# BornToDeath/h264-h265-to-jpeg

Hardware: AMD Instinct MI355X
Metric: 1080p H.265 I-frames/sec → JPEG at 1/2/4/8 MI355X; achieved HBM GB/s vs peak (higher is better)
Workload: dtype u8

## Files before the change

### h264-h265-to-jpeg_amd/csrc/host/cabac.h

```cpp
#pragma once
#include <cstdint>

namespace h2j {

#ifdef H2J_CABAC_COUNT
extern thread_local unsigned long long g_bins_ctx, g_bins_byp;
#define H2J_COUNT(v, n) (v += (n))
#else
#define H2J_COUNT(v, n) ((void)0)
#endif

#pragma GCC visibility push(hidden)
extern const uint8_t kCabacLps[64][4];
extern const uint8_t kCabacTransLps[64];
extern const uint8_t kCabacRenorm[32];
extern const uint16_t kCabacNextMps[128];
extern const uint16_t kCabacNextLps[128];
extern const uint8_t kCabacLpsByState[128][8];
typedef uint64_t CabacState;
extern const uint64_t kCabacWord[128];

extern const uint64_t kCabacNextMpsW[128];
extern const uint64_t kCabacNextLpsW[128];
#pragma GCC visibility pop


inline uint8_t cabac_init_state(int m, int n, int qp) {
    if (qp < 0) qp = 0;
    if (qp > 51) qp = 51;
    int pre = ((m * qp) >> 4) + n;
    if (pre < 1) pre = 1;
    if (pre > 126) pre = 126;
    int mps = pre <= 63 ? 0 : 1;
    int st = mps ? pre - 64 : 63 - pre;
    return static_cast<uint8_t>((st << 1) | mps);
}
inline CabacState cabac_init_word(int m, int n, int qp) { return kCabacWord[cabac_init_state(m, n, qp)]; }

template <bool kInlineRefill>
class CabacT {
public:
    void init(const uint8_t* p, const uint8_t* end) {
        cur_ = p;
        end_ = end;
        range_ = 510;
        value_ = 0;
        for (int i = 0; i < 4; i++) value_ = (value_ << 8) | (cur_ < end_ ? *cur_++ : 0u);
        bits_ = 32 - 9;
    }
    __attribute__((always_inline)) inline int decision(CabacState& ctx) {
        H2J_COUNT(g_bins_ctx, 1);
        const uint64_t w = ctx;
        const unsigned st = static_cast<unsigned>(w >> 32);
        const uint32_t lps = static_cast<uint32_t>(w >> ((range_ >> 3) & 24)) & 0xffu;
        const uint32_t rmps = range_ - lps;
        const uint64_t scaled = static_cast<uint64_t>(rmps) << bits_;
        const uint32_t msh = (rmps >> 8) ^ 1u;
        uint32_t r = rmps << msh, sh = msh;
        const uint32_t lsh = static_cast<uint32_t>(__builtin_clz(lps)) - 23u;
        const uint32_t lr = lps << lsh;
        uint64_t nx = kCabacNextMpsW[st];
        const uint64_t nl = kCabacNextLpsW[st];
        uint64_t v = value_;
        const uint64_t vl = value_ - scaled;
        uint32_t is_lps = 0;
#if defined(__x86_64__)
        __asm__("cmpq %[sc], %[v]\n\t"
                "cmovaeq %[vl], %[v]\n\t"
                "cmovael %[lr], %[r]\n\t"
                "cmovael %[ls], %[sh]\n\t"
                "cmovaeq %[nl], %[nx]\n\t"
                "setae %b[il]"
                : [v] "+r"(v), [r] "+r"(r), [sh] "+r"(sh), [nx] "+r"(nx), [il] "+q"(is_lps)
                : [sc] "r"(scaled), [vl] "r"(vl), [lr] "r"(lr), [ls] "r"(lsh), [nl] "r"(nl)
                : "cc");
#else
        is_lps = v >= scaled ? 1u : 0u;
        v = is_lps ? vl : v;
        r = is_lps ? lr : r;
        sh = is_lps ? lsh : sh;
        nx = is_lps ? nl : nx;
#endif
        value_ = v;
        range_ = r;
        bits_ -= static_cast<int>(sh);
        ctx = nx;
        if (bits_ < 0) refill();
        return static_cast<int>((st & 1) ^ is_lps);
    }
    __attribute__((always_inline)) int bypass_b() {
        H2J_COUNT(g_bins_byp, 1);
        if (--bits_ < 0) refill();
        const uint64_t scaled = static_cast<uint64_t>(range_) << bits_;
        const bool one = value_ >= scaled;
        value_ -= one ? scaled : 0;
        return one;
    }
    __attribute__((always_inline)) uint32_t bypass_batch_b(int k) {
        H2J_COUNT(g_bins_byp, k);
        if (bits_ < k) refill();
        const int sh = bits_ - k;
        const uint64_t v = value_ >> sh;
        const uint32_t q = static_cast<uint32_t>(v / range_);
        value_ -= (static_cast<uint64_t>(q) * range_) << sh;
        bits_ = sh;
        return q;
    }
    __attribute__((always_inline)) uint32_t bypass_peek_b(int k) {
        if (bits_ < k) refill();
        return static_cast<uint32_t>((value_ >> (bits_ - k)) / range_);
    }
    __attribute__((always_inline)) void bypass_skip_b(int n, uint32_t top) {
        H2J_COUNT(g_bins_byp, n);
        const int sh = bits_ - n;
        value_ -= (static_cast<uint64_t>(top) * range_) << sh;
        bits_ = sh;
    }
    __attribute__((always_inline)) uint32_t bypass_bits_b(int n) {
        if (n <= 2) {
            uint32_t v = 0;
            for (int i = 0; i < n; i++) v = (v << 1) | static_cast<uint32_t>(bypass());
            return v;
        }
        if (n <= 24) return bypass_batch(n);
        const uint32_t hi = bypass_batch(n - 16);
        return (hi << 16) | bypass_batch(16);
    }
    __attribute__((always_inline)) int terminate_b() {
        range_ -= 2;
        const uint64_t scaled = static_cast<uint64_t>(range_) << bits_;
        if (value_ >= scaled) return 1;
        if (range_ < 256) {
            range_ <<= 1;
            if (--bits_ < 0) refill();
// ... 64 lines not shown
```

### h264-h265-to-jpeg_amd/csrc/host/hevc_parser.cpp

```cpp
#include <algorithm>
#include <array>
#include <atomic>
#include <cstdlib>
#include <cstring>
#include <memory>
#include <thread>
#include <vector>

#include "bitstream.h"
#include "cabac.h"
#include "job.h"

namespace h2j {
#ifdef H2J_CORO
extern thread_local void (*g_h2j_yield)();
#endif
namespace {

enum {
    C_SAO_MERGE = 0, C_SAO_TYPE = 1, C_SPLIT_CU = 2, C_TQ_BYPASS = 5, C_PART_MODE = 6,
    C_PREV_INTRA = 7, C_CHROMA_MODE = 8, C_SPLIT_TF = 9, C_CBF_LUMA = 12, C_CBF_CHROMA = 14,
    C_TSKIP = 18, C_LAST_X = 20, C_LAST_Y = 38, C_CSBF = 56, C_SIG = 60, C_GT1 = 104,
    C_GT2 = 128, C_QP_DELTA = 134, C_CQO_FLAG = 136, C_CQO_IDX = 137, NUM_CTX = 138
};

const uint8_t kInitI[NUM_CTX] = {
    153, 200, 139, 141, 157, 154, 184, 184, 63, 153, 138, 138, 111, 141, 94, 138, 182, 154,
    139, 139,
    110, 110, 124, 125, 140, 153, 125, 127, 140, 109, 111, 143, 127, 111, 79, 108, 123, 63,
    110, 110, 124, 125, 140, 153, 125, 127, 140, 109, 111, 143, 127, 111, 79, 108, 123, 63,
    91, 171, 134, 141,
    111, 111, 125, 110, 110, 94, 124, 108, 124, 107, 125, 141, 179, 153, 125, 107, 125, 141,
    179, 153, 125, 107, 125, 141, 179, 153, 125, 140, 139, 182, 182, 152, 136, 152, 136, 153,
    136, 139, 111, 136, 139, 111, 141, 111,
    140, 92, 137, 138, 140, 152, 138, 139, 153, 74, 149, 92, 139, 107, 122, 152, 140, 179, 166,
    182, 140, 227, 122, 197,
    138, 153, 136, 167, 152, 152,
    154, 154,
    154, 154};

struct Sps {
    bool valid = false;
    int chroma_format_idc = 0, width = 0, height = 0;
    int conf_l = 0, conf_r = 0, conf_t = 0, conf_b = 0;
    int bit_depth = 8, bit_depth_c = 8, log2_max_poc_lsb = 4;
    int num_reorder_pics = 0;
    int log2_min_cb = 3, log2_ctb = 4, log2_min_tb = 2, log2_max_tb = 5, max_th_depth_intra = 0;
    int scaling_list_enabled = 0;
    uint8_t sl[4][6][64];
    uint8_t sl_dc[4][6];
    int sao = 0, pcm = 0, pcm_bd = 8, pcm_bd_c = 8, log2_min_pcm = 0, log2_max_pcm = 0, pcm_lf_disabled = 0;
    int num_st_rps = 0;
    int st_num_delta[65];
    int long_term_present = 0, num_lt_sps = 0, temporal_mvp = 0, strong_intra_smoothing = 0;
    int profile_idc = 0;
    int ts_rotation = 0, ts_context = 0, implicit_rdpcm = 0, explicit_rdpcm = 0, ext_precision = 0;
    int smoothing_disabled = 0, high_prec_offsets = 0, persistent_rice = 0, bypass_alignment = 0;
};

struct Pps {
    bool valid = false;
    int sps_id = 0, dependent_slices = 0, output_flag_present = 0, num_extra_bits = 0, sign_hiding = 0;
    int init_qp = 26, transform_skip = 0, cu_qp_delta = 0, diff_cu_qp_delta_depth = 0;
    int cb_qp_offset = 0, cr_qp_offset = 0, slice_chroma_qp_present = 0, transquant_bypass = 0;
    int tiles = 0, wpp = 0, ntc = 1, ntr = 1, uniform = 1, lf_across_tiles = 1;
    int col_w[64], row_h[64];
    int lf_across_slices = 0, deblock_override = 0, deblock_disabled = 0, beta_offset = 0, tc_offset = 0;
    int sl_present = 0;
    uint8_t sl[4][6][64];
    uint8_t sl_dc[4][6];
    int slice_header_ext = 0;
    int log2_max_ts = 2, cross_component = 0, cqo_list_enabled = 0, sao_scale_luma = 0, sao_scale_chroma = 0;
    int cqo_depth = 0, cqo_len_minus1 = 0, cb_qo[6] = {0, 0, 0, 0, 0, 0}, cr_qo[6] = {0, 0, 0, 0, 0, 0};
};

struct SliceHdr {
    int first_in_pic = 0, dependent = 0, address = 0, slice_addr_rs = 0, pps_id = 0, type = 0;
    int sao_luma = 0, sao_chroma = 0, qp_delta = 0, cb_qp_offset = 0, cr_qp_offset = 0;
    int deblock_disabled = 0, beta_offset = 0, tc_offset = 0, lf_across_slices = 0, slice_qp = 26;
    int cu_chroma_qp_offset_enabled = 0;
    std::vector<uint32_t> entry;
};

const uint8_t kSlIntra[64] = {
    16, 16, 16, 16, 16, 16, 16, 16, 16, 16, 17, 16, 17, 16, 17, 18, 17, 18, 18, 17, 18, 21,
    19, 20, 21, 20, 19, 21, 24, 22, 22, 24, 24, 22, 22, 24, 25, 25, 27, 30, 27, 25, 25, 29,
    31, 35, 35, 31, 29, 36, 41, 44, 41, 36, 47, 54, 54, 47, 65, 70, 65, 88, 88, 115};
const uint8_t kSlInter[64] = {
    16, 16, 16, 16, 16, 16, 16, 16, 16, 16, 17, 17, 17, 17, 17, 18, 18, 18, 18, 18, 18, 20,
    20, 20, 20, 20, 20, 20, 24, 24, 24, 24, 24, 24, 24, 24, 25, 25, 25, 25, 25, 25, 25, 28,
    28, 28, 28, 28, 28, 33, 33, 33, 33, 33, 41, 41, 41, 41, 54, 54, 54, 71, 71, 91};

void sl_default(uint8_t sl[4][6][64], uint8_t dc[4][6]) {
    for (int m = 0; m < 6; m++) {
        std::memset(sl[0][m], 16, 16);
        for (int s = 1; s < 4; s++) {
            std::memcpy(sl[s][m], m < 3 ? kSlIntra : kSlInter, 64);
            dc[s][m] = 16;
        }
// ... 266 lines not shown
    p.cr_qp_offset = b.se();
    if (p.cb_qp_offset < -12 || p.cb_qp_offset > 12 || p.cr_qp_offset < -12 || p.cr_qp_offset > 12) return -1;
    p.slice_chroma_qp_present = static_cast<int>(b.u(1));
    b.u(1);
    b.u(1);
    p.transquant_bypass = static_cast<int>(b.u(1));
    p.tiles = static_cast<int>(b.u(1));
    p.wpp = static_cast<int>(b.u(1));
    if (p.tiles) {
        const uint32_t ntc = b.ue(), ntr = b.ue();
        if (ntc > 63 || ntr > 63) return -1;
        p.ntc = static_cast<int>(ntc) + 1;
        p.ntr = static_cast<int>(ntr) + 1;
        p.uniform = static_cast<int>(b.u(1));
        if (!p.uniform) {
            for (int i = 0; i < p.ntc - 1; i++) {
                const uint32_t v = b.ue();
                if (v >= 512) return -1;
                p.col_w[i] = static_cast<int>(v) + 1;
            }
            for (int i = 0; i < p.ntr - 1; i++) {
                const uint32_t v = b.ue();
                if (v >= 512) return -1;
                p.row_h[i] = static_cast<int>(v) + 1;
            }
        }
        p.lf_across_tiles = static_cast<int>(b.u(1));
    }
    p.lf_across_slices = static_cast<int>(b.u(1));
    if (b.u(1)) {
        p.deblock_override = static_cast<int>(b.u(1));
        p.deblock_disabled = static_cast<int>(b.u(1));
        if (!p.deblock_disabled) {
            const int bo = b.se(), to = b.se();
            if (bo < -6 || bo > 6 || to < -6 || to > 6) return -1;
            p.beta_offset = bo * 2;
            p.tc_offset = to * 2;
        }
    }
    p.sl_present = static_cast<int>(b.u(1));
    if (p.sl_present) {
        sl_default(p.sl, p.sl_dc);
        parse_scaling_list(b, p.sl, p.sl_dc);
    }
    b.u(1);
    b.ue();
    p.slice_header_ext = static_cast<int>(b.u(1));
    if (b.u(1)) {
        const int range = static_cast<int>(b.u(1));
        b.u(7);
        if (range && sps.profile_idc == 4) {
            if (p.transform_skip) {
                const uint32_t v = b.ue();
                if (v > 3) return -1;
                p.log2_max_ts = static_cast<int>(v) + 2;
            }
            p.cross_component = static_cast<int>(b.u(1));
            p.cqo_list_enabled = static_cast<int>(b.u(1));
            if (p.cqo_list_enabled) {
                p.cqo_depth = static_cast<int>(std::min<uint32_t>(b.ue(), 64u));
                const uint32_t len = b.ue();
                if (len > 5) return -1;
                p.cqo_len_minus1 = static_cast<int>(len);
                for (uint32_t i = 0; i <= len; i++) {
                    p.cb_qo[i] = std::max(-128, std::min(128, b.se()));
                    p.cr_qo[i] = std::max(-128, std::min(128, b.se()));
                }
            }
            const uint32_t sl = b.ue(), sc = b.ue();
            const uint32_t lim = sps.bit_depth > 10 ? static_cast<uint32_t>(sps.bit_depth - 10) : 0u;
            if (sl > lim || sc > lim) return -1;
            p.sao_scale_luma = static_cast<int>(sl);
            p.sao_scale_chroma = static_cast<int>(sc);
        }
    }
    if (b.overrun()) return -1;
    p.valid = true;
    return 0;
}

uint8_t g_scan_diag[4][64][2], g_scan_hor[4][64][2], g_scan_ver[4][64][2];
uint8_t g_scan_inv[3][4][64];
uint16_t g_scan_off[3][4][16];
uint8_t g_diag_pos4[16];
uint8_t g_diag_pos8[64];
uint8_t g_sigctx[2][4][3][4][2][16];
bool g_scans_ready = false;

void init_scans() {
    if (g_scans_ready) return;
    for (int l = 0; l < 4; l++) {
        int bs = 1 << l, i = 0, x = 0, y = 0;
        while (i < bs * bs) {
            while (y >= 0) {
                if (x < bs && y < bs) {
                    g_scan_diag[l][i][0] = static_cast<uint8_t>(x);
                    g_scan_diag[l][i][1] = static_cast<uint8_t>(y);
                    i++;
                }
                y--;
                x++;
            }
            y = x;
            x = 0;
        }
        i = 0;
        for (y = 0; y < bs; y++)
            for (x = 0; x < bs; x++, i++) {
                g_scan_hor[l][i][0] = static_cast<uint8_t>(x);
                g_scan_hor[l][i][1] = static_cast<uint8_t>(y);
            }
        i = 0;
        for (x = 0; x < bs; x++)
            for (y = 0; y < bs; y++, i++) {
                g_scan_ver[l][i][0] = static_cast<uint8_t>(x);
                g_scan_ver[l][i][1] = static_cast<uint8_t>(y);
            }
    }
    for (int si = 0; si < 3; si++)
        for (int l = 0; l < 4; l++) {
            const uint8_t(*sc)[64][2] = si == 0 ? g_scan_diag : (si == 1 ? g_scan_hor : g_scan_ver);
            for (int i = 0; i < (1 << (2 * l)); i++)
                g_scan_inv[si][l][sc[l][i][1] * (1 << l) + sc[l][i][0]] = static_cast<uint8_t>(i);
        }
    for (int c = 0; c < 2; c++)
        for (int lsb = 0; lsb < 4; lsb++)
            for (int si = 0; si < 3; si++)
                for (int pc = 0; pc < 4; pc++)
                    for (int sb = 0; sb < 2; sb++)
                        for (int nn = 0; nn < 16; nn++) {
                            const uint8_t(*sc)[64][2] = si == 0 ? g_scan_diag : (si == 1 ? g_scan_hor : g_scan_ver);
                            const int log2n = lsb + 2, xp = sc[2][nn][0], yp = sc[2][nn][1];
                            int sigCtx;
                            if (log2n == 2) {
                                static const uint8_t m[16] = {0, 1, 4, 5, 2, 3, 4, 5, 6, 6, 8, 8, 7, 7, 8, 8};
                                sigCtx = m[(yp << 2) + xp];
                            } else if (!sb && xp + yp == 0) {
                                sigCtx = 0;
                            } else {
                                if (pc == 0) sigCtx = (xp + yp == 0) ? 2 : (xp + yp < 3) ? 1 : 0;
                                else if (pc == 1) sigCtx = (yp == 0) ? 2 : (yp == 1) ? 1 : 0;
                                else if (pc == 2) sigCtx = (xp == 0) ? 2 : (xp == 1) ? 1 : 0;
                                else sigCtx = 2;
                                if (c == 0) {
                                    if (sb) sigCtx += 3;
                                    sigCtx += (log2n == 3) ? ((si == 0) ? 9 : 15) : 21;
                                } else {
                                    sigCtx += (log2n == 3) ? 9 : 12;
                                }
                            }
                            g_sigctx[c][lsb][si][pc][sb][nn] = static_cast<uint8_t>(C_SIG + (c == 0 ? sigCtx : 27 + sigCtx));
                        }
    for (int si = 0; si < 3; si++) {
        const uint8_t(*sc)[64][2] = si == 0 ? g_scan_diag : (si == 1 ? g_scan_hor : g_scan_ver);
        for (int l = 0; l < 4; l++)
            for (int i = 0; i < 16; i++) g_scan_off[si][l][i] = static_cast<uint16_t>(sc[2][i][1] * (4 << l) + sc[2][i][0]);
    }
    for (int i = 0; i < 16; i++) g_diag_pos4[i] = static_cast<uint8_t>(g_scan_diag[2][i][1] * 4 + g_scan_diag[2][i][0]);
    for (int i = 0; i < 64; i++) g_diag_pos8[i] = static_cast<uint8_t>(g_scan_diag[3][i][1] * 8 + g_scan_diag[3][i][0]);
    g_scans_ready = true;
}

int chroma_qp_table(int qpi) {
    static const int t[14] = {29, 30, 31, 32, 33, 33, 34, 34, 35, 35, 36, 36, 37, 37};
    if (qpi < 30) return qpi;
    if (qpi > 43) return qpi - 6;
    return t[qpi - 30];
}

class HevcParser {
public:
    explicit HevcParser(FrameJob& job) : job_(&job), ctbs_(&job.ctbs) {}
    HevcParser(const HevcParser& proto, FrameJob& job) : HevcParser(proto) {
        job_ = &job;
        ctbs_ = &job.ctbs;
        bind_maps();
    }
    HevcParser(const HevcParser& proto, bool share_maps) : HevcParser(proto) {
        (void)share_maps;
        ctbs_ = proto.ctbs_;
    }
    int run(const uint8_t* data, size_t size, int threads);

private:
    HevcParser(const HevcParser&) = default;
    FrameJob* job_;
    std::vector<h2j_ctb>* ctbs_;
    Sps sps_[16];
    Pps pps_[64];
    const Sps* s_ = nullptr;
    const Pps* p_ = nullptr;
    std::vector<SliceHdr> sh_;
    std::vector<uint8_t> rbsp_;
    std::vector<uint8_t> slice_data_;
    int W = 0, H = 0, log2ctb = 0, ctbs = 0, ctbW = 0, ctbH = 0, nctb = 0, mw = 0, mh = 0;
    int qpbd = 0;
    std::vector<int8_t> qp_store_;
    std::vector<uint8_t> ipm_store_, ctd_store_;
    std::vector<int> addr_store_, slice_store_;
    int8_t* qp_ = nullptr;
    uint8_t *ipm_ = nullptr, *ctd_ = nullptr;
    int *ctb_addr_rs_ = nullptr, *ctb_slice_ = nullptr;
    void bind_maps() {
        qp_ = qp_store_.data();
        ipm_ = ipm_store_.data();
        ctd_ = ctd_store_.data();
        ctb_addr_rs_ = addr_store_.data();
        ctb_slice_ = slice_store_.data();
    }
    std::vector<int> rs2ts_, ts2rs_, tile_id_, col_bd_;
    const SliceHdr* cur_ = nullptr;
    int cur_idx_ = 0;
    Cabac cc_;
    const uint8_t* end_ = nullptr;
    CabacState ctx_[NUM_CTX], ctx_wpp_[NUM_CTX], ctx_ds_[NUM_CTX];
    int stat_[4] = {0, 0, 0, 0}, stat_wpp_[4] = {0, 0, 0, 0}, stat_ds_[4] = {0, 0, 0, 0};
    bool rext_ = false;
    bool have_ds_ = false;
    int qp_y_ = 0, qg_pred_ = 0, qpd_val_ = 0, last_cu_qp_ = 0;
    bool is_qpd_coded_ = false, first_qg_ = true;
    bool cqo_coded_ = false;
    int cu_qo_cb_ = 0, cu_qo_cr_ = 0;
    int cu_bypass_ = 0;
    int cu_tu_begin_ = 0;
    int err_ = 0;

    int parse_slice_header(BitReader& b, int nal_type, SliceHdr& sh, const SliceHdr* prev);
    bool setup_picture();
    bool setup_tiles();
    int decode_slice_data(int shi, const uint8_t* p, const uint8_t* end);
    struct WppRows;
    int decode_wpp_row(int shi, int row, const uint8_t* p, const uint8_t* end, WppRows& w);
    int run_wpp(const std::vector<uint8_t>& seg, const std::vector<uint32_t>& sub, int threads);
    int decode_tile(int shi, int ts0, int ts1, bool last, const uint8_t* p, const uint8_t* end);
    int run_tiles(const std::vector<uint8_t>& seg, const std::vector<uint32_t>& sub, int threads);
    void merge_parts(const std::vector<FrameJob>& part);
    void ctb_start_contexts(int rs, int ts, bool first);
    void init_contexts(int qp) {
        for (int i = 0; i < NUM_CTX; i++) {
            int iv = kInitI[i];
            ctx_[i] = cabac_init_word((iv >> 4) * 5 - 45, ((iv & 15) << 3) - 16, qp);
        }
        std::memset(stat_, 0, sizeof(stat_));
    }
    bool same_region(int xc, int yc, int xn, int yn) const {
        if (xn < 0 || yn < 0 || xn >= W || yn >= H) return false;
        if (((xn ^ xc) | (yn ^ yc)) >> log2ctb == 0) return true;
        int cn = (yn >> log2ctb) * ctbW + (xn >> log2ctb);
        int cc = (yc >> log2ctb) * ctbW + (xc >> log2ctb);
        if (tile_id_[rs2ts_[cn]] != tile_id_[rs2ts_[cc]] || ctb_slice_[cn] < 0) return false;
        return ctb_addr_rs_[cn] == ctb_addr_rs_[cc];
    }
    void qg_start(int xq, int yq);
    void parse_sao(int rx, int ry);
    void coding_quadtree(int x0, int y0, int log2cb, int depth);
    void coding_unit(int x0, int y0, int log2cb);
    void transform_tree(int x0, int y0, int xb, int yb, int log2n, int depth, int blk, int max_depth,
                        int intra_split, int pcb, int pcr, int cm, int cux, int cuy, int log2cb);
    void transform_unit(int x0, int y0, int xb, int yb, int log2n, int blk, int cbf_l, int cbf_cb,
                        int cbf_cr, int cm, int cux, int cuy, int log2cb);
    template <bool RExt>
    void residual(int log2n, int c, int mode, h2j_tu& tu);
    void emit_tu(int x, int y, int log2n, int c, int mode, uint8_t flags, bool cbf, int pred_mode_for_scan);
    void split_ctb_records(size_t first);
    std::vector<h2j_tu> chroma_tmp_;
    uint8_t edge_flags(int x0, int y0) const;
    void pcm_sample(int x0, int y0, int log2cb);
    int qp_wrap(int x) const {
        const int m = 52 + qpbd;
        if (static_cast<unsigned>(x) < static_cast<unsigned>(2 * m)) return x >= m ? x - m : x;
        return x % m;
    }
    static void fill_rows(uint8_t* p, int stride, int rows, int w, uint8_t v) {
        const uint64_t v8 = 0x0101010101010101ull * v;
        for (int y = 0; y < rows; y++, p += stride) {
            if (w == 2) std::memcpy(p, &v8, 2);
            else if (w == 4) std::memcpy(p, &v8, 4);
            else if (w == 8) std::memcpy(p, &v8, 8);
            else if (w == 16) { std::memcpy(p, &v8, 8); std::memcpy(p + 8, &v8, 8); }
            else std::memset(p, v, static_cast<size_t>(w));
        }
    }
    void set_map(uint8_t* m, int x0, int y0, int n, uint8_t v) {
        int ye = std::min((y0 + n) >> 2, mh), xe = std::min((x0 + n) >> 2, mw);
        fill_rows(&m[(y0 >> 2) * mw + (x0 >> 2)], mw, ye - (y0 >> 2), xe - (x0 >> 2), v);
    }
    void set_qp(int x0, int y0, int n, int qp) {
        int ye = std::min((y0 + n) >> 2, mh), xe = std::min((x0 + n) >> 2, mw);
        fill_rows(reinterpret_cast<uint8_t*>(&qp_[(y0 >> 2) * mw + (x0 >> 2)]), mw, ye - (y0 >> 2), xe - (x0 >> 2),
                  static_cast<uint8_t>(qp & 0xFF));
    }
    __attribute__((always_inline)) int dec(int ctx) { return cc_.decision(ctx_[ctx]); }
};

int HevcParser::parse_slice_header(BitReader& b, int nal_type, SliceHdr& sh, const SliceHdr* prev) {
    sh = SliceHdr();
    sh.first_in_pic = static_cast<int>(b.u(1));
    if (nal_type >= 16 && nal_type <= 23) b.u(1);
    const uint32_t pps_id = b.ue();
    if (pps_id > 63 || !pps_[pps_id].valid) return -1;
    sh.pps_id = static_cast<int>(pps_id);
    const Pps& p = pps_[sh.pps_id];
    if (p.sps_id > 15 || !sps_[p.sps_id].valid) return -1;
    const Sps& s = sps_[p.sps_id];
    if (!sh.first_in_pic) {
        if (p.dependent_slices) sh.dependent = static_cast<int>(b.u(1));
        int cs = 1 << s.log2_ctb;
        int n = ((s.width + cs - 1) / cs) * ((s.height + cs - 1) / cs);
        sh.address = static_cast<int>(b.u(ceil_log2(n)));
        if (sh.address >= n) return -1;
    }
    if (sh.dependent) {
        if (!prev) return -1;
        int addr = sh.address, first = sh.first_in_pic;
        sh = *prev;
        sh.address = addr;
        sh.dependent = 1;
        sh.first_in_pic = first;
    } else {
        sh.slice_addr_rs = sh.address;
        for (int i = 0; i < p.num_extra_bits; i++) b.u(1);
        sh.type = static_cast<int>(b.ue());
        if (p.output_flag_present) b.u(1);
        if (nal_type != 19 && nal_type != 20) {
            b.u(s.log2_max_poc_lsb);
            int sps_flag = static_cast<int>(b.u(1));
            if (!sps_flag) {
                Sps tmp = s;
                if (!parse_st_rps(b, tmp, s.num_st_rps)) return -1;
            } else if (s.num_st_rps > 1) {
                b.u(ceil_log2(s.num_st_rps));
            }
            if (s.long_term_present) {
                uint32_t nsps = 0;
                if (s.num_lt_sps > 0) nsps = b.ue();
                const uint32_t npics = b.ue();
                if (nsps > static_cast<uint32_t>(s.num_lt_sps) || npics > 32) return -1;
                for (uint32_t i = 0; i < nsps + npics; i++) {
                    if (i < nsps) {
                        if (s.num_lt_sps > 1) b.u(ceil_log2(s.num_lt_sps));
                    } else {
                        b.u(s.log2_max_poc_lsb);
                        b.u(1);
                    }
// ... 215 lines not shown
        std::memcpy(r.type, o.type, 3);
        std::memcpy(r.band_pos, o.band_pos, 3);
        std::memcpy(r.eo_class, o.eo_class, 3);
        std::memcpy(r.off, o.off, sizeof(r.off));
    };
    if (rx > 0) {
        int l = ctb - 1;
        if (tile_id_[rs2ts_[l]] == tile_id_[rs2ts_[ctb]] && ctb_slice_[l] >= 0 && ctb_addr_rs_[l] == ctb_addr_rs_[ctb]) {
            if (dec(C_SAO_MERGE)) { copy_from(l); return; }
        }
    }
    if (ry > 0) {
        int u = ctb - ctbW;
        if (tile_id_[rs2ts_[u]] == tile_id_[rs2ts_[ctb]] && ctb_slice_[u] >= 0 && ctb_addr_rs_[u] == ctb_addr_rs_[ctb]) {
            if (dec(C_SAO_MERGE)) { copy_from(u); return; }
        }
    }
    const int bd = s_->bit_depth;
    const int cmax = (1 << ((bd < 10 ? bd : 10) - 5)) - 1;
    for (int c = 0; c < 3; c++) {
        if ((c == 0 && !cur_->sao_luma) || (c > 0 && !cur_->sao_chroma)) continue;
        const int shift = c ? p_->sao_scale_chroma : p_->sao_scale_luma;
        if (c == 2) {
            r.type[2] = r.type[1];
            r.eo_class[2] = r.eo_class[1];
        } else {
            int t = 0;
            if (dec(C_SAO_TYPE)) t = cc_.bypass() ? 2 : 1;
            r.type[c] = static_cast<int8_t>(t);
        }
        if (r.type[c] == 0) continue;
        int a[4];
        for (int i = 0; i < 4; i++) {
            int v = 0;
            while (v < cmax && cc_.bypass()) v++;
            a[i] = v;
        }
        if (r.type[c] == 1) {
            for (int i = 0; i < 4; i++)
                if (a[i] && cc_.bypass()) a[i] = -a[i];
            r.band_pos[c] = static_cast<int8_t>(cc_.bypass_bits(5));
            for (int i = 0; i < 4; i++) r.off[c][i] = static_cast<int16_t>(a[i] * (1 << shift));
        } else {
            r.off[c][0] = static_cast<int16_t>(a[0] << shift);
            r.off[c][1] = static_cast<int16_t>(a[1] << shift);
            r.off[c][2] = static_cast<int16_t>(-(a[2] << shift));
            r.off[c][3] = static_cast<int16_t>(-(a[3] << shift));
            if (c == 0) r.eo_class[0] = static_cast<int8_t>(cc_.bypass_bits(2));
            if (c == 1) r.eo_class[1] = static_cast<int8_t>(cc_.bypass_bits(2));
        }
    }
}

uint8_t HevcParser::edge_flags(int x0, int y0) const {
    if (cur_->deblock_disabled) return 0;
    uint8_t f = 0;
    const int mask = ctbs - 1;
    if ((x0 & 7) == 0 && x0 > 0) {
        bool ok = true;
        if ((x0 & mask) == 0) {
            int cn = (y0 >> log2ctb) * ctbW + ((x0 - 1) >> log2ctb), cc = cn + 1;
            if (!cur_->lf_across_slices && ctb_addr_rs_[cn] != ctb_addr_rs_[cc]) ok = false;
            if (!p_->lf_across_tiles && tile_id_[rs2ts_[cn]] != tile_id_[rs2ts_[cc]]) ok = false;
        }
        if (ok) f |= H2J_TU_EDGE_L;
    }
    if ((y0 & 7) == 0 && y0 > 0) {
        bool ok = true;
        if ((y0 & mask) == 0) {
            int cc = (y0 >> log2ctb) * ctbW + (x0 >> log2ctb), cn = cc - ctbW;
            if (!cur_->lf_across_slices && ctb_addr_rs_[cn] != ctb_addr_rs_[cc]) ok = false;
            if (!p_->lf_across_tiles && tile_id_[rs2ts_[cn]] != tile_id_[rs2ts_[cc]]) ok = false;
        }
        if (ok) f |= H2J_TU_EDGE_T;
    }
    return f;
}

const uint8_t kSigTs[2][16] = {{C_SIG + 42, C_SIG + 42, C_SIG + 42, C_SIG + 42, C_SIG + 42, C_SIG + 42, C_SIG + 42, C_SIG + 42,
                                C_SIG + 42, C_SIG + 42, C_SIG + 42, C_SIG + 42, C_SIG + 42, C_SIG + 42, C_SIG + 42, C_SIG + 42},
                               {C_SIG + 43, C_SIG + 43, C_SIG + 43, C_SIG + 43, C_SIG + 43, C_SIG + 43, C_SIG + 43, C_SIG + 43,
                                C_SIG + 43, C_SIG + 43, C_SIG + 43, C_SIG + 43, C_SIG + 43, C_SIG + 43, C_SIG + 43, C_SIG + 43}};

template <bool RExt>
void HevcParser::residual(int log2n, int c, int pred_mode, h2j_tu& tu) {
    Cabac cc = cc_;
    CabacState* const ctx = ctx_;
    const int n = 1 << log2n;
    if (p_->transform_skip && !cu_bypass_ && log2n <= (RExt ? p_->log2_max_ts : 2) && cc.decision(ctx[C_TSKIP + (c ? 1 : 0)]))
        tu.flags |= H2J_TU_TSKIP;
    const bool tsb = (tu.flags & H2J_TU_TSKIP) != 0 || cu_bypass_;
    const bool ts_ctx = RExt && s_->ts_context && tsb;
    const bool no_sdh = RExt && s_->implicit_rdpcm && (tu.flags & H2J_TU_TSKIP) && (pred_mode == 10 || pred_mode == 26);
    const bool price = RExt && s_->persistent_rice;
    int* const stat = &stat_[2 * (c == 0 ? 1 : 0) + (tsb ? 1 : 0)];
    int off, shift;
    if (c == 0) {
        off = 3 * (log2n - 2) + ((log2n - 1) >> 2);
        shift = (log2n + 1) >> 2;
    } else {
        off = 15;
        shift = log2n - 2;
    }
    const int maxp = (log2n << 1) - 1;
    auto last_prefix = [&](CabacState* lc) __attribute__((always_inline)) {
        int k = 0, pk = 0;
        CabacState pw = lc[0];
        while (k < maxp) {
            const int ci = k >> shift;
            const CabacState lw = lc[ci];
            lc[pk] = pw;
            CabacState w = ci == pk ? pw : lw;
            const int b = cc.decision(w);
            pw = w;
            pk = ci;
            if (!b) break;
            k++;
        }
        lc[pk] = pw;
        return k;
    };
    int lx = last_prefix(ctx + C_LAST_X + off);
    int ly = last_prefix(ctx + C_LAST_Y + off);
    if (lx > 3) {
        int nb = (lx >> 1) - 1;
        lx = (1 << nb) * (2 + (lx & 1)) + static_cast<int>(cc.bypass_bits(nb));
    }
    if (ly > 3) {
        int nb = (ly >> 1) - 1;
        ly = (1 << nb) * (2 + (ly & 1)) + static_cast<int>(cc.bypass_bits(nb));
    }
    int scanIdx = 0;
    if (log2n == 2 || (log2n == 3 && c == 0)) {
        if (pred_mode >= 6 && pred_mode <= 14) scanIdx = 2;
        else if (pred_mode >= 22 && pred_mode <= 30) scanIdx = 1;
    }
    if (scanIdx == 2) std::swap(lx, ly);
    if (lx >= n || ly >= n) { err_ = -20; cc_ = cc; return; }
    const uint8_t(*sc)[64][2] = scanIdx == 0 ? g_scan_diag : (scanIdx == 1 ? g_scan_hor : g_scan_ver);
    const int lsb = log2n - 2;
    const int lastSub = g_scan_inv[scanIdx][lsb][((ly >> 2) << lsb) + (lx >> 2)];
    const int lastPos = g_scan_inv[scanIdx][2][((ly & 3) << 2) + (lx & 3)];
    uint8_t csbf[8][8];
    std::memset(csbf, 0, sizeof(csbf));
    int greater1_ctx = 1;
    const bool sdh = p_->sign_hiding != 0;
    const int sbw = 1 << lsb;
    uint32_t out[32 * 32];
    int nout = 0;
    const uint16_t* const posTab = g_scan_off[scanIdx][lsb];
    const uint8_t(*const sigtab)[2][16] = g_sigctx[c ? 1 : 0][lsb][scanIdx];
    CabacState* const gt1ctx = ctx + C_GT1 + (c ? 16 : 0);
    for (int i = lastSub; i >= 0; i--) {
#ifdef H2J_CORO_SB
        if (i < lastSub && g_h2j_yield) g_h2j_yield();
#endif
        const int xs = sc[lsb][i][0], ys = sc[lsb][i][1];
        bool infer_dc = false;
        if (i < lastSub && i > 0) {
            int csr = (xs + 1 < sbw) ? csbf[xs + 1][ys] : 0;
            int csb = (ys + 1 < sbw) ? csbf[xs][ys + 1] : 0;
            csbf[xs][ys] = static_cast<uint8_t>(cc.decision(ctx[C_CSBF + (csr | csb) + (c ? 2 : 0)]));
            infer_dc = true;
        } else {
            csbf[xs][ys] = 1;
        }
        unsigned sigmask = 0;
        int nstart = 15;
        if (i == lastSub) {
            nstart = lastPos - 1;
            sigmask = 1u << lastPos;
        }
        if (csbf[xs][ys]) {
            int prevCsbf = 0;
            if (xs + 1 < sbw) prevCsbf |= csbf[xs + 1][ys];
            if (ys + 1 < sbw) prevCsbf |= csbf[xs][ys + 1] << 1;
            const uint8_t* sig = ts_ctx ? kSigTs[c ? 1 : 0] : sigtab[prevCsbf][(xs | ys) ? 1 : 0];
            unsigned got = 0;
            if (nstart > 0) {
                int pidx = sig[nstart];
                CabacState pw = ctx[pidx];
                got = static_cast<unsigned>(cc.decision(pw)) << nstart;
                for (int nn = nstart - 1; nn > 0; nn--) {
                    const int idx = sig[nn];
                    const CabacState lw = ctx[idx];
                    ctx[pidx] = pw;
                    CabacState w = idx == pidx ? pw : lw;
                    got |= static_cast<unsigned>(cc.decision(w)) << nn;
                    pw = w;
                    pidx = idx;
                }
                ctx[pidx] = pw;
            }
            sigmask |= got;
            infer_dc = infer_dc && got == 0;
            if (nstart >= 0) {
                if (!infer_dc) {
                    if (cc.decision(ctx[sig[0]])) sigmask |= 1u;
                } else {
                    sigmask |= 1u;
                }
            }
        }
        if (!sigmask) continue;
        int ctxSet = (i == 0 || c > 0) ? 0 : 2;
        if (greater1_ctx == 0) ctxSet++;
        greater1_ctx = 1;
        unsigned g1mask = 0;
        int numG1 = 0, lastG1 = -1;
        unsigned m_uncoded = 0;
        const int lastSig = 31 - __builtin_clz(sigmask), firstSig = __builtin_ctz(sigmask);
        CabacState* const g1c = gt1ctx + ctxSet * 4;
        {
            CabacState w0 = g1c[0], w1 = g1c[1], w2 = g1c[2], w3 = g1c[3];
            unsigned seen = 0, m = sigmask;
            auto bin = [&](CabacState& slot) __attribute__((always_inline)) {
                const int nn = 31 - __builtin_clz(m);
                m &= ~(1u << nn);
                CabacState w = seen ? w0 : slot;
                const unsigned d = static_cast<unsigned>(cc.decision(w));
                if (seen) w0 = w;
                else slot = w;
                seen |= d;
                g1mask |= d << nn;
                numG1++;
            };
            if (m) bin(w1);
            if (m) bin(w2);
            while (m && numG1 < 8) bin(w3);
            g1c[0] = w0;
            g1c[1] = w1;
            g1c[2] = w2;
            g1c[3] = w3;
            m_uncoded = m;
            greater1_ctx = seen ? 0 : 1;
        }
        if (g1mask) lastG1 = 31 - __builtin_clz(g1mask);
        const bool hidden = !cu_bypass_ && !no_sdh && (lastSig - firstSig > 3);
        int g2 = 0;
        if (lastG1 != -1) g2 = cc.decision(ctx[C_GT2 + ctxSet + (c ? 4 : 0)]);
        const unsigned signed_mask = (sdh && hidden) ? (sigmask & ~(1u << firstSig)) : sigmask;
        const int ns = __builtin_popcount(signed_mask);
        const uint32_t q = ns > 1 ? cc.bypass_batch(ns) : (ns ? static_cast<uint32_t>(cc.bypass()) : 0u);
        uint32_t qs = ns ? q << (32 - ns) : 0u;
        unsigned esc = g1mask | m_uncoded;
        if (lastG1 >= 0 && !g2) esc &= ~(1u << lastG1);
        int remv[16] = {};
        int rice = price ? *stat / 4 : 0;
        bool stat_done = false;
        for (unsigned e = esc; e;) {
            const int nn = 31 - __builtin_clz(e);
            e &= ~(1u << nn);
            const int baseL = 1 + ((g1mask >> nn) & 1) + (nn == lastG1 ? g2 : 0);
            {
                constexpr int kPeek = 20;
                const uint32_t q = cc.bypass_peek(kPeek);
                const uint32_t inv = ~q << (32 - kPeek);
                int prefix = inv ? __builtin_clz(inv) : kPeek;
                int rem = -1;
                if (prefix < kPeek) {
                    const int slen = prefix < 3 ? rice : prefix - 3 + rice, total = prefix + 1 + slen;
                    if (total <= kPeek) {
                        const uint32_t top = q >> (kPeek - total);
                        cc.bypass_skip(total, top);
                        const int suf = static_cast<int>(top & ((1u << slen) - 1u));
                        rem = prefix < 3 ? (prefix << rice) + suf : (((1 << (prefix - 3)) + 2) << rice) + suf;
                    }
                }
                if (rem < 0) {
                    prefix = 0;
                    while (prefix < 32 && cc.bypass()) prefix++;
                    if (prefix < 3) rem = (prefix << rice) + static_cast<int>(cc.bypass_bits(rice));
                    else {
                        int pm3 = prefix - 3;
                        if (pm3 + rice > 30) { err_ = -21; cc_ = cc; return; }
                        rem = (((1 << pm3) + 2) << rice) + static_cast<int>(cc.bypass_bits(pm3 + rice));
                    }
                }
                remv[nn] = rem;
                if (baseL + rem > 3 * (1 << rice)) rice = price ? rice + 1 : (rice < 4 ? rice + 1 : 4);
                if (price && !stat_done) {
                    const int ri = *stat / 4;
                    if (rem >= (3 << ri)) ++*stat;
                    else if (2 * rem < (1 << ri) && *stat > 0) --*stat;
                    stat_done = true;
                }
            }
        }
        const int flip_last = (sdh && hidden) ? 1 : 0;
        const int sb_off = ((ys << 2) << log2n) + (xs << 2);
        int sumAbs = 0;
        for (unsigned mm = sigmask; mm;) {
            const int nn = 31 - __builtin_clz(mm);
            mm &= ~(1u << nn);
            const int lvl = 1 + ((g1mask >> nn) & 1) + (nn == lastG1 ? g2 : 0) + remv[nn];
            sumAbs += lvl;
            const int neg = static_cast<int>(qs >> 31) ^ (mm == 0 ? (flip_last & sumAbs) : 0);
            qs <<= 1;
            int v = neg ? -lvl : lvl;
            if (v > 32767) v = 32767;
            if (v < -32768) v = -32768;
            out[nout++] = (static_cast<uint32_t>(sb_off + posTab[nn]) << 16) | static_cast<uint16_t>(v);
        }
    }
    cc_ = cc;
    const uint32_t base = static_cast<uint32_t>(job_->coefs.size());
    job_->coefs.insert(job_->coefs.end(), out, out + nout);
    tu.coef = base - job_->hdr.coef;
    tu.ncoef = static_cast<uint16_t>(nout);
    tu.flags |= H2J_TU_CBF;
}

void HevcParser::split_ctb_records(size_t first) {
    std::vector<h2j_tu>& v = job_->tus;
    chroma_tmp_.clear();
    size_t w = first;
    for (size_t i = first; i < v.size(); i++) {
        if (v[i].c == 0) v[w++] = v[i];
        else chroma_tmp_.push_back(v[i]);
    }
    std::copy(chroma_tmp_.begin(), chroma_tmp_.end(), v.begin() + static_cast<long>(w));
}

void HevcParser::emit_tu(int x, int y, int log2n, int c, int mode, uint8_t flags, bool cbf, int) {
    job_->tus.emplace_back();
    h2j_tu& tu = job_->tus.back();
    tu.x = static_cast<uint16_t>(x);
    tu.y = static_cast<uint16_t>(y);
    tu.log2n = static_cast<uint8_t>(log2n);
    tu.c = static_cast<uint8_t>(c);
    tu.mode = static_cast<uint8_t>(mode);
    tu.flags = flags;
    tu.qp = 0;
    tu.qpy = 0;
    tu.ncoef = 0;
    tu.coef = 0;
    if (cbf) {
#ifdef H2J_CORO
        if (g_h2j_yield) g_h2j_yield();
#endif
        if (rext_) residual<true>(log2n, c, mode, tu);
        else residual<false>(log2n, c, mode, tu);
    }
}

void HevcParser::transform_unit(int x0, int y0, int xb, int yb, int log2n, int blk, int cbf_l, int cbf_cb,
                                int cbf_cr, int cm, int cux, int cuy, int log2cb) {
    if ((cbf_l || cbf_cb || cbf_cr) && p_->cu_qp_delta && !is_qpd_coded_) {
        int v = 0;
        if (dec(C_QP_DELTA)) {
            v = 1;
            while (v < 5 && dec(C_QP_DELTA + 1)) v++;
            if (v == 5) {
                int k = 0;
                while (k < 32 && cc_.bypass()) k++;
                if (k > 30) { err_ = -22; return; }
                v += ((1 << k) - 1) + static_cast<int>(cc_.bypass_bits(k));
            }
        }
        if (v && cc_.bypass()) v = -v;
        is_qpd_coded_ = true;
        qpd_val_ = v;
        qp_y_ = qp_wrap(qg_pred_ + v + 52 + 2 * qpbd) - qpbd;
        set_qp(cux, cuy, 1 << log2cb, qp_y_);
    }
    if ((cbf_cb || cbf_cr) && cur_->cu_chroma_qp_offset_enabled && !cu_bypass_ && !cqo_coded_) {
        int idx = -1;
        if (dec(C_CQO_FLAG)) {
            idx = 0;
            if (p_->cqo_len_minus1 > 0)
                while (idx < 5 && dec(C_CQO_IDX)) idx++;
        }
        cu_qo_cb_ = idx < 0 ? 0 : p_->cb_qo[idx];
        cu_qo_cr_ = idx < 0 ? 0 : p_->cr_qo[idx];
        cqo_coded_ = true;
    }
    const int lmode = ipm_[(y0 >> 2) * mw + (x0 >> 2)];
    uint8_t fl = edge_flags(x0, y0);
    if (cu_bypass_) fl |= H2J_TU_BYPASS | H2J_TU_NOFILT;
    uint8_t lfl = fl;
    if (log2n == 2) lfl |= H2J_TU_DST;
    emit_tu(x0, y0, log2n, 0, lmode, lfl, cbf_l != 0, lmode);
    if ((job_->tus.back().flags & (H2J_TU_TSKIP | H2J_TU_BYPASS)) != 0) job_->tus.back().flags &= ~H2J_TU_DST;
    if (err_) return;
    uint8_t cfl = cu_bypass_ ? (H2J_TU_BYPASS | H2J_TU_NOFILT) : 0;
    if (log2n > 2) {
        emit_tu(x0 >> 1, y0 >> 1, log2n - 1, 1, cm, cfl, cbf_cb != 0, cm);
        if (err_) return;
        emit_tu(x0 >> 1, y0 >> 1, log2n - 1, 2, cm, cfl, cbf_cr != 0, cm);
    } else if (blk == 3) {
        emit_tu(xb >> 1, yb >> 1, 2, 1, cm, cfl, cbf_cb != 0, cm);
        if (err_) return;
        emit_tu(xb >> 1, yb >> 1, 2, 2, cm, cfl, cbf_cr != 0, cm);
    }
}

void HevcParser::transform_tree(int x0, int y0, int xb, int yb, int log2n, int depth, int blk, int max_depth,
                                int intra_split, int pcb, int pcr, int cm, int cux, int cuy, int log2cb) {
    if (err_) return;
    int split;
    if (log2n <= s_->log2_max_tb && log2n > s_->log2_min_tb && depth < max_depth && !(intra_split && depth == 0))
        split = dec(C_SPLIT_TF + 5 - log2n);
    else
        split = log2n > s_->log2_max_tb || (intra_split && depth == 0);
    int cbf_cb = 0, cbf_cr = 0;
    if (log2n > 2) {
        if (depth == 0 || pcb) cbf_cb = dec(C_CBF_CHROMA + depth);
        if (depth == 0 || pcr) cbf_cr = dec(C_CBF_CHROMA + depth);
    } else {
        cbf_cb = pcb;
        cbf_cr = pcr;
    }
    if (split) {
        if (log2n <= 2) { err_ = -23; return; }
        int h = 1 << (log2n - 1);
        transform_tree(x0, y0, x0, y0, log2n - 1, depth + 1, 0, max_depth, intra_split, cbf_cb, cbf_cr, cm, cux, cuy, log2cb);
        transform_tree(x0 + h, y0, x0, y0, log2n - 1, depth + 1, 1, max_depth, intra_split, cbf_cb, cbf_cr, cm, cux, cuy, log2cb);
        transform_tree(x0, y0 + h, x0, y0, log2n - 1, depth + 1, 2, max_depth, intra_split, cbf_cb, cbf_cr, cm, cux, cuy, log2cb);
        transform_tree(x0 + h, y0 + h, x0, y0, log2n - 1, depth + 1, 3, max_depth, intra_split, cbf_cb, cbf_cr, cm, cux, cuy, log2cb);
    } else {
        int cbf_l = dec(C_CBF_LUMA + (depth == 0 ? 1 : 0));
        transform_unit(x0, y0, xb, yb, log2n, blk, cbf_l, cbf_cb, cbf_cr, cm, cux, cuy, log2cb);
    }
}

// ... 573 lines not shown
```

Baseline: 1985.

## Specialize 4x4 residual decode path and vectorize coefficient level reconstruction with AVX2

Adds a Small template specialization of the HEVC residual parser for 4x4 TUs. It drops the subblock flag logic, the memset and the bypass suffix handling, and writes coefficients straight into the job vector instead of a staging buffer. It also replaces the scalar per-coefficient level/sign loop with AVX2 mask expansion, pdep sign scatter and a compress-store through a permute table. The coroutine yield hooks are removed and per-class bin counters are added for profiling. The host CABAC parse is the target cost; the risks are correctness of the SIMD sign-hiding parity and the AVX2 stores writing up to 8 entries past nout.

After: 1919. 3.4% lower.

```diff
diff --git a/h264-h265-to-jpeg_amd/csrc/host/cabac.h b/h264-h265-to-jpeg_amd/csrc/host/cabac.h
--- a/h264-h265-to-jpeg_amd/csrc/host/cabac.h
+++ b/h264-h265-to-jpeg_amd/csrc/host/cabac.h
@@ -5,9 +5,16 @@
 
 #ifdef H2J_CABAC_COUNT
 extern thread_local unsigned long long g_bins_ctx, g_bins_byp;
+enum { H2J_BIN_OTHER = 0, H2J_BIN_SIG, H2J_BIN_CSBF, H2J_BIN_LAST, H2J_BIN_GT1, H2J_BIN_GT2, H2J_BIN_CLASSES };
+extern thread_local unsigned long long g_bins_class[H2J_BIN_CLASSES];
+extern thread_local int g_bin_class;
 #define H2J_COUNT(v, n) (v += (n))
+#define H2J_COUNT_CTX() (g_bins_ctx++, g_bins_class[g_bin_class]++)
+#define H2J_BIN_CLASS(k) (g_bin_class = (k))
 #else
 #define H2J_COUNT(v, n) ((void)0)
+#define H2J_COUNT_CTX() ((void)0)
+#define H2J_BIN_CLASS(k) ((void)0)
 #endif
 
 #pragma GCC visibility push(hidden)
@@ -49,7 +56,7 @@
         bits_ = 32 - 9;
     }
     __attribute__((always_inline)) inline int decision(CabacState& ctx) {
-        H2J_COUNT(g_bins_ctx, 1);
+        H2J_COUNT_CTX();
         const uint64_t w = ctx;
         const unsigned st = static_cast<unsigned>(w >> 32);
         const uint32_t lps = static_cast<uint32_t>(w >> ((range_ >> 3) & 24)) & 0xffu;
diff --git a/h264-h265-to-jpeg_amd/csrc/host/hevc_parser.cpp b/h264-h265-to-jpeg_amd/csrc/host/hevc_parser.cpp
--- a/h264-h265-to-jpeg_amd/csrc/host/hevc_parser.cpp
+++ b/h264-h265-to-jpeg_amd/csrc/host/hevc_parser.cpp
@@ -11,10 +11,14 @@
 #include "cabac.h"
 #include "job.h"
 
+#if defined(__AVX2__) && defined(__BMI2__) && defined(__POPCNT__)
+#include <immintrin.h>
+#define H2J_SIMD_LEVELS 1
+#else
+#define H2J_SIMD_LEVELS 0
+#endif
+
 namespace h2j {
-#ifdef H2J_CORO
-extern thread_local void (*g_h2j_yield)();
-#endif
 namespace {
 
 enum {
@@ -447,6 +451,8 @@
 uint8_t g_scan_diag[4][64][2], g_scan_hor[4][64][2], g_scan_ver[4][64][2];
 uint8_t g_scan_inv[3][4][64];
 uint16_t g_scan_off[3][4][16];
+alignas(32) uint32_t g_scan_ent[3][4][16];
+alignas(8) uint8_t g_pack8[256][8];
 uint8_t g_diag_pos4[16];
 uint8_t g_diag_pos8[64];
 uint8_t g_sigctx[2][4][3][4][2][16];
@@ -519,8 +525,14 @@
     for (int si = 0; si < 3; si++) {
         const uint8_t(*sc)[64][2] = si == 0 ? g_scan_diag : (si == 1 ? g_scan_hor : g_scan_ver);
         for (int l = 0; l < 4; l++)
-            for (int i = 0; i < 16; i++) g_scan_off[si][l][i] = static_cast<uint16_t>(sc[2][i][1] * (4 << l) + sc[2][i][0]);
-    }
+            for (int i = 0; i < 16; i++) {
+                g_scan_off[si][l][i] = static_cast<uint16_t>(sc[2][i][1] * (4 << l) + sc[2][i][0]);
+                g_scan_ent[si][l][15 - i] = static_cast<uint32_t>(g_scan_off[si][l][i]) << 16;
+            }
+    }
+    for (int m = 0; m < 256; m++)
+        for (int j = 0, k = 0; j < 8; j++)
+            if (m >> j & 1) g_pack8[m][k++] = static_cast<uint8_t>(j);
     for (int i = 0; i < 16; i++) g_diag_pos4[i] = static_cast<uint8_t>(g_scan_diag[2][i][1] * 4 + g_scan_diag[2][i][0]);
     for (int i = 0; i < 64; i++) g_diag_pos8[i] = static_cast<uint8_t>(g_scan_diag[3][i][1] * 8 + g_scan_diag[3][i][0]);
     g_scans_ready = true;
@@ -624,7 +636,7 @@
                         int intra_split, int pcb, int pcr, int cm, int cux, int cuy, int log2cb);
     void transform_unit(int x0, int y0, int xb, int yb, int log2n, int blk, int cbf_l, int cbf_cb,
                         int cbf_cr, int cm, int cux, int cuy, int log2cb);
-    template <bool RExt>
+    template <bool RExt, bool Small>
     void residual(int log2n, int c, int mode, h2j_tu& tu);
     void emit_tu(int x, int y, int log2n, int c, int mode, uint8_t flags, bool cbf, int pred_mode_for_scan);
     void split_ctb_records(size_t first);
@@ -1006,11 +1018,14 @@
                                {C_SIG + 43, C_SIG + 43, C_SIG + 43, C_SIG + 43, C_SIG + 43, C_SIG + 43, C_SIG + 43, C_SIG + 43,
                                 C_SIG + 43, C_SIG + 43, C_SIG + 43, C_SIG + 43, C_SIG + 43, C_SIG + 43, C_SIG + 43, C_SIG + 43}};
 
-template <bool RExt>
-void HevcParser::residual(int log2n, int c, int pred_mode, h2j_tu& tu) {
+template <bool RExt, bool Small>
+void HevcParser::residual(int log2n_arg, int c, int pred_mode, h2j_tu& tu) {
+    static_assert(!(RExt && Small), "the 4x4 path is v1 only");
     Cabac cc = cc_;
     CabacState* const ctx = ctx_;
+    const int log2n = Small ? 2 : log2n_arg;
     const int n = 1 << log2n;
+    H2J_BIN_CLASS(H2J_BIN_OTHER);
     if (p_->transform_skip && !cu_bypass_ && log2n <= (RExt ? p_->log2_max_ts : 2) && cc.decision(ctx[C_TSKIP + (c ? 1 : 0)]))
         tu.flags |= H2J_TU_TSKIP;
     const bool tsb = (tu.flags & H2J_TU_TSKIP) != 0 || cu_bypass_;
@@ -1028,6 +1043,11 @@
     }
     const int maxp = (log2n << 1) - 1;
     auto last_prefix = [&](CabacState* lc) __attribute__((always_inline)) {
+        if (Small) {
+            int k = 0;
+            while (k < 3 && cc.decision(lc[k])) k++;
+            return k;
+        }
         int k = 0, pk = 0;
         CabacState pw = lc[0];
         while (k < maxp) {
@@ -1044,18 +1064,20 @@
         lc[pk] = pw;
         return k;
     };
+    H2J_BIN_CLASS(H2J_BIN_LAST);
     int lx = last_prefix(ctx + C_LAST_X + off);
     int ly = last_prefix(ctx + C_LAST_Y + off);
-    if (lx > 3) {
+    H2J_BIN_CLASS(H2J_BIN_OTHER);
+    if (!Small && lx > 3) {
         int nb = (lx >> 1) - 1;
         lx = (1 << nb) * (2 + (lx & 1)) + static_cast<int>(cc.bypass_bits(nb));
     }
-    if (ly > 3) {
+    if (!Small && ly > 3) {
         int nb = (ly >> 1) - 1;
         ly = (1 << nb) * (2 + (ly & 1)) + static_cast<int>(cc.bypass_bits(nb));
     }
     int scanIdx = 0;
-    if (log2n == 2 || (log2n == 3 && c == 0)) {
+    if (Small || log2n == 2 || (log2n == 3 && c == 0)) {
         if (pred_mode >= 6 && pred_mode <= 14) scanIdx = 2;
         else if (pred_mode >= 22 && pred_mode <= 30) scanIdx = 1;
     }
@@ -1063,39 +1085,66 @@
     if (lx >= n || ly >= n) { err_ = -20; cc_ = cc; return; }
     const uint8_t(*sc)[64][2] = scanIdx == 0 ? g_scan_diag : (scanIdx == 1 ? g_scan_hor : g_scan_ver);
     const int lsb = log2n - 2;
-    const int lastSub = g_scan_inv[scanIdx][lsb][((ly >> 2) << lsb) + (lx >> 2)];
+    const int lastSub = Small ? 0 : g_scan_inv[scanIdx][lsb][((ly >> 2) << lsb) + (lx >> 2)];
     const int lastPos = g_scan_inv[scanIdx][2][((ly & 3) << 2) + (lx & 3)];
     uint8_t csbf[8][8];
-    std::memset(csbf, 0, sizeof(csbf));
+    if (!Small) std::memset(csbf, 0, sizeof(csbf));
     int greater1_ctx = 1;
     const bool sdh = p_->sign_hiding != 0;
     const int sbw = 1 << lsb;
-    uint32_t out[32 * 32];
+    const size_t cbase = job_->coefs.size();
+    uint32_t outbuf[Small ? 1 : 32 * 32];
+    uint32_t* out = outbuf;
+    if (Small) {
+        job_->coefs.resize(cbase + 16);
+        out = job_->coefs.data() + cbase;
+    }
     int nout = 0;
     const uint16_t* const posTab = g_scan_off[scanIdx][lsb];
     const uint8_t(*const sigtab)[2][16] = g_sigctx[c ? 1 : 0][lsb][scanIdx];
     CabacState* const gt1ctx = ctx + C_GT1 + (c ? 16 : 0);
     for (int i = lastSub; i >= 0; i--) {
-#ifdef H2J_CORO_SB
-        if (i < lastSub && g_h2j_yield) g_h2j_yield();
-#endif
-        const int xs = sc[lsb][i][0], ys = sc[lsb][i][1];
+        const int xs = Small ? 0 : sc[lsb][i][0], ys = Small ? 0 : sc[lsb][i][1];
         bool infer_dc = false;
-        if (i < lastSub && i > 0) {
-            int csr = (xs + 1 < sbw) ? csbf[xs + 1][ys] : 0;
-            int csb = (ys + 1 < sbw) ? csbf[xs][ys + 1] : 0;
-            csbf[xs][ys] = static_cast<uint8_t>(cc.decision(ctx[C_CSBF + (csr | csb) + (c ? 2 : 0)]));
-            infer_dc = true;
-        } else {
-            csbf[xs][ys] = 1;
+        bool coded = true;
+        if (!Small) {
+            if (i < lastSub && i > 0) {
+                int csr = (xs + 1 < sbw) ? csbf[xs + 1][ys] : 0;
+                int csb = (ys + 1 < sbw) ? csbf[xs][ys + 1] : 0;
+                H2J_BIN_CLASS(H2J_BIN_CSBF);
+                csbf[xs][ys] = static_cast<uint8_t>(cc.decision(ctx[C_CSBF + (csr | csb) + (c ? 2 : 0)]));
+                infer_dc = true;
+            } else {
+                csbf[xs][ys] = 1;
+            }
+            coded = csbf[xs][ys] != 0;
         }
         unsigned sigmask = 0;
         int nstart = 15;
-        if (i == lastSub) {
+        if (Small || i == lastSub) {
             nstart = lastPos - 1;
             sigmask = 1u << lastPos;
         }
-        if (csbf[xs][ys]) {
+        H2J_BIN_CLASS(H2J_BIN_SIG);
+        if (Small) {
+            const uint8_t* sig = sigtab[0][0];
+            if (nstart >= 0) {
+                int pidx = sig[nstart];
+                CabacState pw = ctx[pidx];
+                unsigned got = static_cast<unsigned>(cc.decision(pw)) << nstart;
+                for (int nn = nstart - 1; nn >= 0; nn--) {
+                    const int idx = sig[nn];
+                    const CabacState lw = ctx[idx];
+                    ctx[pidx] = pw;
+                    CabacState w = idx == pidx ? pw : lw;
+                    got |= static_cast<unsigned>(cc.decision(w)) << nn;
+                    pw = w;
+                    pidx = idx;
+                }
+                ctx[pidx] = pw;
+                sigmask |= got;
+            }
+        } else if (coded) {
             int prevCsbf = 0;
             if (xs + 1 < sbw) prevCsbf |= csbf[xs + 1][ys];
             if (ys + 1 < sbw) prevCsbf |= csbf[xs][ys + 1] << 1;
@@ -1126,9 +1175,10 @@
                 }
             }
         }
-        if (!sigmask) continue;
+        if (!Small && !sigmask) continue;
+        H2J_BIN_CLASS(H2J_BIN_GT1);
         int ctxSet = (i == 0 || c > 0) ? 0 : 2;
-        if (greater1_ctx == 0) ctxSet++;
+        if (!Small && greater1_ctx == 0) ctxSet++;
         greater1_ctx = 1;
         unsigned g1mask = 0;
         int numG1 = 0, lastG1 = -1;
@@ -1162,14 +1212,17 @@
         if (g1mask) lastG1 = 31 - __builtin_clz(g1mask);
         const bool hidden = !cu_bypass_ && !no_sdh && (lastSig - firstSig > 3);
         int g2 = 0;
+        H2J_BIN_CLASS(H2J_BIN_GT2);
         if (lastG1 != -1) g2 = cc.decision(ctx[C_GT2 + ctxSet + (c ? 4 : 0)]);
+        H2J_BIN_CLASS(H2J_BIN_OTHER);
         const unsigned signed_mask = (sdh && hidden) ? (sigmask & ~(1u << firstSig)) : sigmask;
         const int ns = __builtin_popcount(signed_mask);
         const uint32_t q = ns > 1 ? cc.bypass_batch(ns) : (ns ? static_cast<uint32_t>(cc.bypass()) : 0u);
         uint32_t qs = ns ? q << (32 - ns) : 0u;
         unsigned esc = g1mask | m_uncoded;
         if (lastG1 >= 0 && !g2) esc &= ~(1u << lastG1);
-        int remv[16] = {};
+        constexpr int kRemRev = H2J_SIMD_LEVELS ? 15 : 0;
+        alignas(32) int remv[16] = {};
         int rice = price ? *stat / 4 : 0;
         bool stat_done = false;
         for (unsigned e = esc; e;) {
@@ -1197,11 +1250,16 @@
                     if (prefix < 3) rem = (prefix << rice) + static_cast<int>(cc.bypass_bits(rice));
                     else {
                         int pm3 = prefix - 3;
-                        if (pm3 + rice > 30) { err_ = -21; cc_ = cc; return; }
+                        if (pm3 + rice > 30) {
+                            err_ = -21;
+                            cc_ = cc;
+                            if (Small) job_->coefs.resize(cbase);
+                            return;
+                        }
                         rem = (((1 << pm3) + 2) << rice) + static_cast<int>(cc.bypass_bits(pm3 + rice));
                     }
                 }
-                remv[nn] = rem;
+                remv[nn ^ kRemRev] = rem;
                 if (baseL + rem > 3 * (1 << rice)) rice = price ? rice + 1 : (rice < 4 ? rice + 1 : 4);
                 if (price && !stat_done) {
                     const int ri = *stat / 4;
@@ -1213,6 +1271,51 @@
         }
         const int flip_last = (sdh && hidden) ? 1 : 0;
         const int sb_off = ((ys << 2) << log2n) + (xs << 2);
+#if H2J_SIMD_LEVELS
+        {
+            const __m256i bit_hi = _mm256_setr_epi32(1 << 15, 1 << 14, 1 << 13, 1 << 12, 1 << 11, 1 << 10, 1 << 9, 1 << 8);
+            const __m256i bit_lo = _mm256_setr_epi32(1 << 7, 1 << 6, 1 << 5, 1 << 4, 1 << 3, 1 << 2, 1 << 1, 1);
+            const __m256i one = _mm256_set1_epi32(1);
+            const __m256i g2v = _mm256_set1_epi32(static_cast<int>(static_cast<unsigned>(g2) << (lastG1 & 15)));
+            const __m256i sigv = _mm256_set1_epi32(static_cast<int>(sigmask)), g1v = _mm256_set1_epi32(static_cast<int>(g1mask));
+            const __m256i sig_hi = _mm256_cmpeq_epi32(_mm256_and_si256(sigv, bit_hi), bit_hi);
+            const __m256i sig_lo = _mm256_cmpeq_epi32(_mm256_and_si256(sigv, bit_lo), bit_lo);
+            const __m256i g1_hi = _mm256_add_epi32(_mm256_cmpeq_epi32(_mm256_and_si256(g1v, bit_hi), bit_hi),
+                                                   _mm256_cmpeq_epi32(_mm256_and_si256(g2v, bit_hi), bit_hi));
+            const __m256i g1_lo = _mm256_add_epi32(_mm256_cmpeq_epi32(_mm256_and_si256(g1v, bit_lo), bit_lo),
+                                                   _mm256_cmpeq_epi32(_mm256_and_si256(g2v, bit_lo), bit_lo));
+            const __m256i rem_hi = _mm256_load_si256(reinterpret_cast<const __m256i*>(remv));
+            const __m256i rem_lo = _mm256_load_si256(reinterpret_cast<const __m256i*>(remv + 8));
+            const __m256i lvl_hi = _mm256_and_si256(sig_hi, _mm256_sub_epi32(_mm256_add_epi32(one, rem_hi), g1_hi));
+            const __m256i lvl_lo = _mm256_and_si256(sig_lo, _mm256_sub_epi32(_mm256_add_epi32(one, rem_lo), g1_lo));
+            const unsigned odd = static_cast<unsigned>(_mm256_movemask_ps(_mm256_castsi256_ps(_mm256_slli_epi32(lvl_hi, 31)))) ^
+                                 static_cast<unsigned>(_mm256_movemask_ps(_mm256_castsi256_ps(_mm256_slli_epi32(lvl_lo, 31))));
+            const unsigned parity = static_cast<unsigned>(_mm_popcnt_u32(odd)) & 1u;
+            const unsigned negmask = _pdep_u32(q, signed_mask) | ((static_cast<unsigned>(flip_last) & parity) << firstSig);
+            const __m256i negv = _mm256_set1_epi32(static_cast<int>(negmask));
+            const __m256i neg_hi = _mm256_cmpeq_epi32(_mm256_and_si256(negv, bit_hi), bit_hi);
+            const __m256i neg_lo = _mm256_cmpeq_epi32(_mm256_and_si256(negv, bit_lo), bit_lo);
+            const __m256i lim_hi = _mm256_set1_epi32(32767), lim_lo = _mm256_set1_epi32(-32768);
+            __m256i v_hi = _mm256_sub_epi32(_mm256_xor_si256(lvl_hi, neg_hi), neg_hi);
+            __m256i v_lo = _mm256_sub_epi32(_mm256_xor_si256(lvl_lo, neg_lo), neg_lo);
+            v_hi = _mm256_max_epi32(_mm256_min_epi32(v_hi, lim_hi), lim_lo);
+            v_lo = _mm256_max_epi32(_mm256_min_epi32(v_lo, lim_hi), lim_lo);
+            const __m256i low16 = _mm256_set1_epi32(0xffff), sbv = _mm256_set1_epi32(sb_off << 16);
+            const __m256i* const ent = reinterpret_cast<const __m256i*>(g_scan_ent[scanIdx][lsb]);
+            const __m256i e_hi = _mm256_or_si256(_mm256_and_si256(v_hi, low16), _mm256_add_epi32(_mm256_load_si256(ent), sbv));
+            const __m256i e_lo = _mm256_or_si256(_mm256_and_si256(v_lo, low16), _mm256_add_epi32(_mm256_load_si256(ent + 1), sbv));
+            const unsigned m_hi = static_cast<unsigned>(_mm256_movemask_ps(_mm256_castsi256_ps(sig_hi)));
+            const unsigned m_lo = static_cast<unsigned>(_mm256_movemask_ps(_mm256_castsi256_ps(sig_lo)));
+            const __m256i p_hi = _mm256_cvtepu8_epi32(_mm_loadl_epi64(reinterpret_cast<const __m128i*>(g_pack8[m_hi])));
+            const __m256i p_lo = _mm256_cvtepu8_epi32(_mm_loadl_epi64(reinterpret_cast<const __m128i*>(g_pack8[m_lo])));
+            _mm256_storeu_si256(reinterpret_cast<__m256i*>(out + nout), _mm256_permutevar8x32_epi32(e_hi, p_hi));
+            nout += _mm_popcnt_u32(m_hi);
+            _mm256_storeu_si256(reinterpret_cast<__m256i*>(out + nout), _mm256_permutevar8x32_epi32(e_lo, p_lo));
+            nout += _mm_popcnt_u32(m_lo);
+            (void)qs;
+            (void)posTab;
+        }
+#else
         int sumAbs = 0;
         for (unsigned mm = sigmask; mm;) {
             const int nn = 31 - __builtin_clz(mm);
@@ -1226,10 +1329,13 @@
             if (v < -32768) v = -32768;
             out[nout++] = (static_cast<uint32_t>(sb_off + posTab[nn]) << 16) | static_cast<uint16_t>(v);
         }
+#endif
     }
     cc_ = cc;
-    const uint32_t base = static_cast<uint32_t>(job_->coefs.size());
-    job_->coefs.insert(job_->coefs.end(), out, out + nout);
+    H2J_BIN_CLASS(H2J_BIN_OTHER);
+    const uint32_t base = static_cast<uint32_t>(cbase);
+    if (Small) job_->coefs.resize(cbase + static_cast<size_t>(nout));
+    else job_->coefs.insert(job_->coefs.end(), out, out + nout);
     tu.coef = base - job_->hdr.coef;
     tu.ncoef = static_cast<uint16_t>(nout);
     tu.flags |= H2J_TU_CBF;
@@ -1260,11 +1366,9 @@
     tu.ncoef = 0;
     tu.coef = 0;
     if (cbf) {
-#ifdef H2J_CORO
-        if (g_h2j_yield) g_h2j_yield();
-#endif
-        if (rext_) residual<true>(log2n, c, mode, tu);
-        else residual<false>(log2n, c, mode, tu);
+        if (rext_) residual<true, false>(log2n, c, mode, tu);
+        else if (log2n == 2) residual<false, true>(2, c, mode, tu);
+        else residual<false, false>(log2n, c, mode, tu);
     }
 }
 
```
